# gfacciol/mgm

Measured on AMD Instinct MI355X. Metric: disparity-volumes/sec (W*H*L cost volume -> 8-dir MGM -> WTA+vfit), higher is better.
Workload: dtype f32

## Files before the change

mgm_amd/csrc/mgm_pass.hip:

```cpp
#include "mgm_pass_common.h"

namespace mgm {

template <int LPL, bool FH, bool WEIGHTED, int R>
__global__ void __launch_bounds__(R * 64) k_pass(const PassParams P)
{
    constexpr int LP = LPL * 64;
    constexpr int NS = (WEIGHTED && !FH) ? 2 : 1;
    using NbT = Nb<LPL, NS>;
    extern __shared__ __attribute__((aligned(16))) float smem[];
    float *ring = smem;
    float *ringm = smem + R * 2 * NS * LP;
    int *s_task = reinterpret_cast<int *>(ringm + R * 2);

    const int tid = threadIdx.x, lane = tid & 63;
    const int r = __builtin_amdgcn_readfirstlane(tid >> 6);
    if (tid == 0) *s_task = (int)atomicAdd(P.ticket, 1u);
    __syncthreads();
    const int2 tk = P.tasks[*s_task];
    const int vp = tk.x, band = tk.y;
    const int pass = vp & (kMaxDirs - 1);
    const PassVolume &V = P.vol[vp / kMaxDirs];
    const PassGeom &g = P.g[pass];
    const int NL = g.NL, LL = g.LL, L = P.L, MGM = P.MGM, form = g.form;
// ... 96 lines not shown
                        if (form == 0) combine_unit<LPL>(Cpf[u], nb_i, nb_s, nb_b, nb_f, MGM, FH, Lv);
                        else combine_unit<LPL>(Cpf[u], nb_f, nb_b, nb_s, nb_i, MGM, FH, Lv);
                    } else {
                        float D[4];
#pragma unroll
                        for (int k = 0; k < 4; k++) D[k] = V.w8[(long long)g.wplane[k] * P.npix + pix];
                        int rl = 0, rh = 0x7fffffff;
                        if (FH && V.rlo) {
                            rl = (int)V.rlo[pix] - P.dmin;
                            rh = (int)V.rhi[pix] - P.dmin;
                        }
                        if constexpr (!FH) {
                            if (form == 0) combine_whirsch<LPL>(Cpf[u], nb_i, nb_s, nb_b, nb_f, D, P1, P2, MGM, Lv);
                            else combine_whirsch<LPL>(Cpf[u], nb_f, nb_b, nb_s, nb_i, D, P1, P2, MGM, Lv);
                        } else {
                            if (form == 0) combine_wfh<LPL>(Cpf[u], nb_i, nb_s, nb_b, nb_f, D, P1, P2, MGM, lane, L, Lv, rl, rh);
                            else combine_wfh<LPL>(Cpf[u], nb_f, nb_b, nb_s, nb_i, D, P1, P2, MGM, lane, L, Lv, rl, rh);
                        }
                    }
                } else {
#pragma unroll
                    for (int k = 0; k < LPL; k++) Lv[k] = Cpf[u][k];
                }
                store_slab<LPL>(Lrb + pix * L, lane, L, exact, Lv);

                const float m = slab_min<LPL>(Lv);
                nb_i.m = m;
                if constexpr (!WEIGHTED) {
                    if constexpr (!FH) {
                        float N[LPL];
                        neighbour_min<LPL>(Lv, N);
                        const float cap = m + P2;
#pragma unroll
                        for (int k = 0; k < LPL; k++) nb_i.w[0][k] = fminf(fminf(Lv[k], N[k] + P1), cap);
                    } else {
#pragma unroll
                        for (int k = 0; k < LPL; k++) nb_i.w[0][k] = Lv[k];
                        fh_minconv<LPL>(nb_i.w[0], m, P1, P2, lane, L);
                    }
                } else {
#pragma unroll
                    for (int k = 0; k < LPL; k++) nb_i.w[0][k] = Lv[k];
                    if constexpr (!FH) neighbour_min<LPL>(Lv, nb_i.w[NS - 1]);
                }
                if (to_lds) {
                    float *dst = ring + (r * 2 + (i & 1)) * NS * LP + lane * LPL;
#pragma unroll
                    for (int q = 0; q < NS; q++)
#pragma unroll
                        for (int k = 0; k < LPL; k++) dst[q * LP + k] = nb_i.w[q][k];
                    if (lane == 0) ringm[r * 2 + (i & 1)] = m;
                }
                if (to_global) {
#pragma unroll
                    for (int q = 0; q < NS; q++)
                        store_slab_sc1<LPL>(hand_out + ((long long)i * NS + q) * LP, lane, nb_i.w[q]);
                    if (lane == 0)
                        __hip_atomic_store(reinterpret_cast<unsigned *>(handm_out + i), __builtin_bit_cast(unsigned, m),
                                           RLX_AGENT);
                    if (((i + 1) % CH) == 0 || i == LL - 1) {
                        asm volatile("s_waitcnt vmcnt(0)" ::: "memory");
                        if (lane == 0) __hip_atomic_store(prog_out, (unsigned)(i + 1), RLX_AGENT);
                    }
                }
            }

            issue_prefetch(s + PF, Cpf[u], Hpf[u]);

            lds_barrier();
        }
    }
}

__global__ void __launch_bounds__(256) k_selftest_div3(unsigned long long *nbad)
{
    unsigned long long bad = 0;
    const unsigned long long stride = (unsigned long long)gridDim.x * blockDim.x;
    for (unsigned long long b = (unsigned long long)blockIdx.x * blockDim.x + threadIdx.x; b < (1ull << 32); b += stride) {
        const float x = __builtin_bit_cast(float, (unsigned)b);
        const unsigned a = __builtin_bit_cast(unsigned, x / 3.0f);
        const unsigned q = __builtin_bit_cast(unsigned, div3_exact(x));
        const bool a_nan = (a & 0x7fffffffu) > 0x7f800000u, q_nan = (q & 0x7fffffffu) > 0x7f800000u;
        if (a != q && !(a_nan && q_nan)) bad++;
    }
    if (bad) atomicAdd(nbad, bad);
}
hipError_t launch_selftest_div3(unsigned long long *nbad, hipStream_t s)
{
    hipLaunchKernelGGL(k_selftest_div3, dim3(4096), dim3(256), 0, s, nbad);
    return hipGetLastError();
}

int pass_ns(bool fh, bool weighted) { return (weighted && !fh) ? 2 : 1; }
int pass_lpl(int L)
{
    const int lpl = (L + 63) / 64;
    if (lpl == 5) return 6;
    if (lpl == 7) return 8;
    if (lpl <= 8) return lpl;
    return lpl <= 12 ? 12 : (lpl <= 16 ? 16 : (lpl <= 24 ? 24 : 32));
}

hipError_t launch_pass(const PassParams &p, const PassKernelChoice &c, int ntasks, hipStream_t s)
{
    if (c.family != kPassFirst) return hipErrorInvalidValue;
    return lift<kR, 4>(c.R, [&](auto R) { return lift<32, 24, 16, 12, 8, 6, 4, 3, 2, 1>(c.LPL, [&](auto LPL) { return lift<1, 0>(c.WEIGHTED, [&](auto W) { return lift<0, 1>(c.FH, [&](auto FH) {
        if constexpr (pass_instance(LPL(), R())) {
            auto kern = k_pass<LPL(), FH() != 0, W() != 0, R()>;
            if (c.lds > 48 * 1024) {
                hipError_t e = hipFuncSetAttribute(reinterpret_cast<const void *>(kern), hipFuncAttributeMaxDynamicSharedMemorySize, c.lds);
                if (e != hipSuccess) return e;
            }
            hipLaunchKernelGGL(kern, dim3(ntasks), dim3(c.block), c.lds, s, p);
            return hipGetLastError();
        } else
            return hipErrorInvalidValue;
    }); }); }); });
}

}
```

mgm_amd/csrc/mgm_pass2.hip:

```cpp
#include <type_traits>

#include "mgm_pass_common.h"

namespace mgm {

typedef __attribute__((address_space(3))) void *lds_vptr;
typedef const __attribute__((address_space(1))) void *glb_vptr;

template <int AUX>
__device__ __forceinline__ void dma16(const float *src_lane, float *dst_base)
{
    __builtin_amdgcn_global_load_lds((glb_vptr)src_lane, (lds_vptr)dst_base, 16, 0, AUX);
}
template <int AUX>
__device__ __forceinline__ void dma4(const void *src_lane, void *dst_base)
{
    __builtin_amdgcn_global_load_lds((glb_vptr)src_lane, (lds_vptr)dst_base, 4, 0, AUX);
}
constexpr int AUX_SC1 = 16;

template <int N>
__device__ __forceinline__ void wait_vmcnt()
{
    static_assert(N >= 0 && N <= 63, "vmcnt is a 6-bit counter");
// ... 91 lines not shown
#endif
#ifndef MGM_P2_DEV
#define MGM_P2_DEV 0
#endif

#ifndef MGM_P2_TIMELINE
#define MGM_P2_TIMELINE 0
#endif
#ifndef MGM_P2_C8_NL
#define MGM_P2_C8_NL 1
#endif
#ifndef MGM_P2_C8_NC
#define MGM_P2_C8_NC (16 - MGM_P2_C8_NL)
#endif
#ifndef MGM_P2_MAXD
#define MGM_P2_MAXD 2
#endif
#ifndef MGM_P2_DEEPD
#define MGM_P2_DEEPD 4
#endif
#ifndef MGM_P2_PUBLAG
#define MGM_P2_PUBLAG 3
#endif
#ifndef MGM_P2_PUBEVERY
#define MGM_P2_PUBEVERY 4
#endif
#ifndef MGM_P2_LEAD
#define MGM_P2_LEAD 2
#endif
template <int LPL, int NS, bool HASM, int C8, int MAXD = MGM_P2_MAXD, int EXTRA = 0>
struct Plan {
    static constexpr int LP = LPL * 64;
    static constexpr int IPS = (LPL * 16 + 63) / 64;
    static constexpr int LPS = LPL * 4 * (C8 ? C8 : 1);
    static constexpr int LPD = C8 ? 64 / LPS : 1;
    static constexpr int NL = (LPL <= 4 && MGM_P2_NC > 7) ? (C8 ? MGM_P2_C8_NL : 2) : 1;
    static constexpr int NC = (LPL <= 4) ? (C8 ? MGM_P2_C8_NC : MGM_P2_NC) : 7;
    static constexpr int NCA = (NL == 2) ? NC / 2 : NC;
    static constexpr int NDMA = C8 ? (NC + LPD - 1) / LPD : NCA * IPS;
    static constexpr int nA = ((C8 && NL == 2) ? 0 : NDMA) + NS * IPS + (HASM ? 2 : 0) + EXTRA;
    static constexpr int nB = (C8 && NL == 2) ? NDMA : (NC - NCA) * IPS;
    static constexpr int cring_floats(int rdepth) { return C8 ? rdepth * NDMA * 256 : NC * rdepth * LP; }
    static constexpr int lds_floats3(int rt, int rdepth)
    {
        return NC * rt * NS * LP
               + NC * rt
               + rdepth * NS * LP
               + 2 * rdepth + 8 + 32
               + cring_floats(rdepth)
               + (C8 ? rdepth * 16 : 0)
               + EXTRA * rdepth * 64;
    }
    static constexpr bool fits(int rt, int rdepth, int d)
    {
        return d >= 2 && d <= rdepth - 1 && lds_floats3(rt, rdepth) * 4 <= ((C8 && LPL <= 4 && NS == 1) ? MGM_P2_LDS_KB : 160) * 1024 &&
               nA * (d - 1) <= 63 && nB * (d - 1) <= 63;
    }
    static constexpr int pick(int what)
    {
        const int rts[2] = {2, 2};
        const int rds[3] = {MAXD + 1, 4, 3};
        for (int a = 0; a < 2; a++)
            for (int b = 0; b < 3; b++)
                for (int d = MAXD; d >= 2; d--)
                    if (fits(rts[a], rds[b], d)) return what == 0 ? rts[a] : (what == 1 ? rds[b] : d);
        return 0;
    }
    static constexpr int RT = pick(0), RDEPTH = pick(1), D = pick(2);
    static constexpr int rd(int) { return RDEPTH; }
    static constexpr int lds_floats(int) { return lds_floats3(RT, RDEPTH); }
    static_assert(D >= 2, "no feasible pipeline depth");
    static_assert(!C8 || LPD >= 1, "a compact slab must fit a DMA piece");
    static_assert((RT & (RT - 1)) == 0, "RT must be a power of two");
};

template <int LPL, int MGM, bool FH>
__device__ __forceinline__ void combine_unit_E(const float (&C)[LPL], const float (&e1)[LPL], const float (&e2)[LPL],
                                               const float (&e3)[LPL], const float (&e4)[LPL], float (&out)[LPL])
{
    if constexpr (MGM == 2) {
#pragma unroll
        for (int k = 0; k < LPL; k++) out[k] = C[k] + (e1[k] + e2[k]);
    } else {
#pragma unroll
        for (int k = 0; k < LPL; k++) {
            float e = e1[k];
            if constexpr (MGM >= 3) e += e2[k];
            if constexpr (MGM >= 3) e += e3[k];
            if constexpr (MGM >= 4) e += e4[k];
            out[k] = C[k] + div_small<MGM>(e);
        }
    }
}

template <int LPL, int MGM>
__device__ __forceinline__ void combine_w2(const float (&C)[LPL], const Nb<LPL, 2> &n1, const Nb<LPL, 2> &n2, const Nb<LPL, 2> &n3,
                                           const Nb<LPL, 2> &n4, bool a1, bool a2, bool a3, bool a4, float (&out)[LPL])
{
#pragma unroll
    for (int k = 0; k < LPL; k++) {
        float e = a1 ? n1.w[1][k] : n1.w[0][k];
        if constexpr (MGM >= 2) e += a2 ? n2.w[1][k] : n2.w[0][k];
        if constexpr (MGM >= 3) e += a3 ? n3.w[1][k] : n3.w[0][k];
        if constexpr (MGM >= 4) e += a4 ? n4.w[1][k] : n4.w[0][k];
        out[k] = C[k] + div_small<MGM>(e);
    }
}

template <int LPL, bool FH, bool WEIGHTED, int MGM, int C8, bool DEEP, bool W2 = false>
struct P2Lds {
    static constexpr int NS = (W2 || (WEIGHTED && !FH)) ? 2 : 1;
    static constexpr bool pubE = W2 || (!WEIGHTED && !(FH && MGM == 2));
    using PL = Plan<LPL, NS, !pubE, C8, DEEP ? MGM_P2_DEEPD : MGM_P2_MAXD, W2 ? 1 : 0>;
    static constexpr int RD = PL::rd(PL::D);
    static constexpr int task_off = PL::NC * PL::RT * NS * PL::LP + RD * NS * PL::LP + PL::cring_floats(RD) + PL::NC * PL::RT + RD + RD;
};

template <int LPL, bool FH, bool WEIGHTED, int MGM, int C8, int SUBV, bool DEEP, bool XCDQ, bool W2 = false>
__device__ __forceinline__ void pass2_item(const PassParams &P, const int ticket)
{
    static_assert(!W2 || (!WEIGHTED && C8 && DEEP && SUBV == 1 && LPL <= 4), "two-valued weights: the compact kernels with deep rings");
    static_assert(!DEEP || (C8 && !WEIGHTED && (W2 || !(FH && MGM == 2))), "the deep rings exist for the compact kernels that publish E");
    static_assert(SUBV == 1 || (LPL == 4 && C8 == 1 && !WEIGHTED && !(FH && MGM == 2)), "volumes share a wave only in the compact unweighted kernels that publish E");
    static_assert(!W2 || C8 == 1, "two-valued weights: one byte per cost");
    constexpr int LANES = 64 / SUBV;
    constexpr int NS = (W2 || (WEIGHTED && !FH)) ? 2 : 1;
    constexpr bool pubE = W2 || (!WEIGHTED && !(FH && MGM == 2));
    constexpr bool TAGS = pubE;
    constexpr bool CFLAG = C8 && FH;
    constexpr bool CHMIN = LPL == 4 && SUBV == 1 && C8 == 1 && !WEIGHTED && !W2 && pubE;
    using PL = Plan<LPL, NS, !pubE, C8, DEEP ? MGM_P2_DEEPD : MGM_P2_MAXD, W2 ? 1 : 0>;
    static_assert(!W2 || PL::NL == 1, "two-valued weights: one loader wave");
    constexpr int LP = PL::LP, NC = PL::NC, NCA = PL::NCA, D = PL::D, IPS = PL::IPS;
    constexpr int LPS = PL::LPS, LPD = PL::LPD, NDMA = PL::NDMA;
    constexpr int LPW = NCA;
    constexpr int RD = PL::rd(D);
    constexpr int RT = PL::RT;
    using NbT = Nb<LPL, NS>;

    extern __shared__ __attribute__((aligned(16))) float smem[];
    float *Tring = smem;
    float *Hring = Tring + NC * RT * NS * LP;
    float *Cring = Hring + RD * NS * LP;
    float *Tm = Cring + PL::cring_floats(RD);
    float *Hm = Tm + NC * RT;
    unsigned *Hprog = reinterpret_cast<unsigned *>(Hm + RD);
    int *s_task = reinterpret_cast<int *>(smem + P2Lds<LPL, FH, WEIGHTED, MGM, C8, DEEP, W2>::task_off);
    unsigned *Cflag = reinterpret_cast<unsigned *>(s_task + 40);
    unsigned *Wring = Cflag + RD * 16;

    const int tid = threadIdx.x, lane = tid & 63;
    const int wave = __builtin_amdgcn_readfirstlane(tid >> 6);
    const int2 tk = P.tasks[ticket];
    const int vp = tk.x, band = tk.y & 0xffff, strip = (tk.y >> 16) & 0xff;
    const bool plain_out = XCDQ && ((tk.y >> 24) & 1) != 0;
    const int pass = vp & (kMaxDirs - 1);
    const int vgrp = (vp / kMaxDirs) * SUBV;
    const PassVolume &V = P.vol[vgrp];
#if MGM_P2_DEV
    unsigned long long *dbg = P.dbg ? P.dbg + (long long)ticket * 16 : nullptr;
    const int xflags = P.xflags;
#else
    constexpr unsigned long long *dbg = nullptr;
    constexpr int xflags = 0;
#endif
    if (dbg && tid == 0) dbg[0] = wall_clock64();
    const PassGeom &g = P.g[pass];
    const int NLn = g.NL, LL = g.LL, L = P.L, form = g.form;
    const float P1 = P.P1, P2 = P.P2;
    const int SL = g.slope;
    const bool strips = TAGS && g.nstrips == 2;
    const bool mirror = strips && strip == 1;
    const long long istep = mirror ? -g.istep : g.istep;
    const long long gbase = mirror ? g.base + (long long)(LL - 1) * g.istep : g.base;
    const int W = !strips ? LL : min(LL, (strip == 0 ? g.split : LL - g.split) + NC - 1);
    const int nsteps = ((W + 1 + SL * (NC - 1)) + 2) / 3 * 3;
    const bool from_global = band > 0;

    constexpr int NSLP = NS * LP;
    const long long hslab = (long long)(vp / kMaxDirs) * P.hand_vstride + g.hand_base;
    float *hand_out = TAGS ? P.hand + (hslab + (long long)band * LL) * NSLP : P.hand + ((long long)(vp * 2 + (band & 1)) * P.LLmax) * NSLP;
    float *handm_out = P.handm + (long long)(vp * 2 + (band & 1)) * P.LLmax;
    const float *hand_in = TAGS ? P.hand + (hslab + (long long)(band > 0 ? band - 1 : 0) * LL) * NSLP
                                : P.hand + ((long long)(vp * 2 + ((band + 1) & 1)) * P.LLmax) * NSLP;
    const float *handm_in = P.handm + (long long)(vp * 2 + ((band + 1) & 1)) * P.LLmax;
    unsigned *prog_out = P.prog + vp * P.maxbands + band;
    const unsigned *prog_in = from_global ? prog_out - 1 : prog_out;

    const unsigned tag_in = P.hand_tag[pass], tag_out = tag_in;

    if (wave >= NC) {
        const int wl = wave - NC;
        const int r0 = wl == 0 ? 0 : NCA;
        unsigned known = 0;
        bool dead = false;
        unsigned long long n_slow = 0, t_slow = 0, n_spin = 0, t_ret = 0, t_bar = 0, t_iss = 0, tl_wait = 0;
        (void)tl_wait;
        (void)n_slow;
        (void)n_spin;

        constexpr int NPIECE = C8 ? NDMA : LPW;
        const float *cptr[NPIECE];
        int ci[NPIECE];
        const long long cstride = C8 ? (istep * L * C8) / 4 : istep * L;
#pragma unroll
        for (int q = 0; q < NPIECE; q++) {
            int r = C8 ? q * LPD + lane / LPS : r0 + q;
            r = r < NC ? r : NC - 1;
            int j = band * NC + r;
            j = j < NLn ? j : NLn - 1;
            if constexpr (C8 && SUBV > 1) {
                constexpr int CPV = LPS / SUBV;
                const int chunk = lane % LPS;
// ... 345 lines not shown
                    }
                } else {
                    const float *src = c_src0 + cslot * LP;
#pragma unroll
                    for (int k = 0; k < LPL; k++) Cv[k] = src[k];
                }
                const bool interior = has_prev && i >= 1 && i <= LL - 2;
                if (prof) {
                    asm volatile("s_waitcnt lgkmcnt(0)" ::: "memory");
                    asm volatile("" : "+v"(Cv[0]), "+v"(X.w[0][0]));
                    ph[0] += clock64() - c0;
                }
                const unsigned long long c1 = prof ? clock64() : 0;
                const NbT &nb_same = SLOPE == 2 ? Z : X;
                const NbT &nb_back = SLOPE == 2 ? Y : Z;
                const NbT &nb_fwd = X;
                if (interior) {
                    if constexpr (W2) {
                        const unsigned wm = (unsigned)__builtin_amdgcn_readfirstlane((int)Wring[cslot * 64 + r]);
                        const bool a0 = (wm >> wb[0]) & 1u, a1 = (wm >> wb[1]) & 1u, a2 = (wm >> wb[2]) & 1u, a3 = (wm >> wb[3]) & 1u;
                        if constexpr (FORM == 0) combine_w2<LPL, MGM>(Cv, nb_i, nb_same, nb_back, nb_fwd, a0, a1, a2, a3, Lv);
                        else combine_w2<LPL, MGM>(Cv, nb_fwd, nb_back, nb_same, nb_i, a0, a1, a2, a3, Lv);
                    } else if constexpr (!WEIGHTED) {
                        if constexpr (pubE) {
                            if constexpr (FORM == 0)
                                combine_unit_E<LPL, MGM, FH>(Cv, nb_i.w[0], nb_same.w[0], nb_back.w[0], nb_fwd.w[0], Lv);
                            else
                                combine_unit_E<LPL, MGM, FH>(Cv, nb_fwd.w[0], nb_back.w[0], nb_same.w[0], nb_i.w[0], Lv);
                        } else {
                            if constexpr (FORM == 0) combine_unit<LPL>(Cv, nb_i, nb_same, nb_back, nb_fwd, MGM, FH, Lv);
                            else combine_unit<LPL>(Cv, nb_fwd, nb_back, nb_same, nb_i, MGM, FH, Lv);
                        }
                    } else {
                        float Dw[4];
#pragma unroll
                        for (int k = 0; k < 4; k++) Dw[k] = V.w8[(long long)g.wplane[k] * P.npix + pix];
                        int rl = 0, rh = 0x7fffffff;
                        if (FH && V.rlo) {
                            rl = (int)V.rlo[pix] - P.dmin;
                            rh = (int)V.rhi[pix] - P.dmin;
                        }
                        if constexpr (!FH) {
                            if constexpr (FORM == 0)
                                combine_whirsch<LPL>(Cv, nb_i, nb_same, nb_back, nb_fwd, Dw, P1, P2, MGM, Lv);
                            else
                                combine_whirsch<LPL>(Cv, nb_fwd, nb_back, nb_same, nb_i, Dw, P1, P2, MGM, Lv);
                        } else {
                            if (MGM == 2 && P.fh2_ragged) {
                                if constexpr (FORM == 0) combine_fh2_ragged<LPL>(Cv, nb_i, nb_same, P1, P2, lane, P.Lreal, rl, rh, Lv);
                                else combine_fh2_ragged<LPL>(Cv, nb_fwd, nb_back, P1, P2, lane, P.Lreal, rl, rh, Lv);
                            } else if constexpr (FORM == 0)
                                combine_wfh<LPL>(Cv, nb_i, nb_same, nb_back, nb_fwd, Dw, P1, P2, MGM, lane, P.Lreal, Lv, rl, rh);
                            else
                                combine_wfh<LPL>(Cv, nb_fwd, nb_back, nb_same, nb_i, Dw, P1, P2, MGM, lane, P.Lreal, Lv, rl, rh);
                        }
                    }
                } else {
#pragma unroll
                    for (int k = 0; k < LPL; k++) Lv[k] = Cv[k];
                }
                if (prof) {
                    asm volatile("" : "+v"(Lv[0]), "+v"(Lv[LPL - 1]));
                    ph[1] += clock64() - c1;
                }
                const unsigned long long c2 = prof ? clock64() : 0;
                if (!(xflags & 1)) {
#ifdef MGM_P2_XFLAG16
                    float *q = Lrb + ((xflags & 16) ? (pix & 255) : pix) * L + (lane % LANES) * LPL;
#else
                    float *q = q_here;
#endif
#pragma unroll
                    for (int k = 0; k < LPL; k++) q[k] = Lv[k];
                }
                float m;
                if constexpr (CHMIN) {
                    m = Lv[0];
#pragma unroll
                    for (int k = 1; k < LPL; k++) m = fminf(m, Lv[k]);
                    m = dpp_min_row_shr1(m, m);
                    m = dpp_min_row_shr2(m, m);
                    m = dpp_min_row_shr4(m, m);
                    if (P.min_k != 0 && (lane & 7) == 7)
                        *reinterpret_cast<float *>((long long)(reinterpret_cast<unsigned long long>(q_here) >> 5) + P.min_k) = m;
                    m = dpp_min_row_shr8(m, m);
                    m = dpp_min_bcast15(m, m);
                    m = dpp_min_bcast31(m, m);
                    m = readlane_f(m, 63);
                } else if constexpr (SUBV == 1) {
                    m = slab_min<LPL>(Lv);
                } else {
                    m = Lv[0];
#pragma unroll
                    for (int k = 1; k < LPL; k++) m = fminf(m, Lv[k]);
                    m = dpp_min_row_shr1(m, m);
                    m = dpp_min_row_shr2(m, m);
                    m = dpp_min_row_shr4(m, m);
                    m = dpp_min_row_shr8(m, m);
                    if constexpr (SUBV == 2) m = dpp_min_bcast15(m, m);
                    m = __shfl(m, lane | (LANES - 1));
                }
                nb_i.m = m;
                if (prof) {
                    float mm = m;
                    asm volatile("" : "+v"(mm));
                    ph[2] += clock64() - c2;
                }
                const unsigned long long c3 = prof ? clock64() : 0;
                if constexpr (W2) {
                    const float P1a = V.p1a, P2a = V.p2a;
                    if constexpr (!FH) {
                        float N[LPL];
                        neighbour_min<LPL>(Lv, N);
                        const float cap = m + P2, capa = m + P2a;
#pragma unroll
                        for (int k = 0; k < LPL; k++) {
                            nb_i.w[0][k] = fminf(fminf(Lv[k], N[k] + P1), cap) - m;
                            nb_i.w[1][k] = fminf(fminf(Lv[k], N[k] + P1a), capa) - m;
                        }
                    } else {
#pragma unroll
                        for (int k = 0; k < LPL; k++) nb_i.w[0][k] = nb_i.w[1][k] = Lv[k];
                        unsigned sw = 0;
                        const unsigned need = ((unsigned)__builtin_amdgcn_readfirstlane((int)Wring[cslot * 64 + r]) >> (8 + 2 * pass)) & 3u;
                        if (need & 1u) fh_minconv<LPL, false, 1>(nb_i.w[0], m, P1, P2, lane, P.Lreal, sw);
                        if (need & 2u) fh_minconv<LPL, false, 1>(nb_i.w[1], m, P1a, P2a, lane, P.Lreal, sw);
#pragma unroll
                        for (int k = 0; k < LPL; k++) {
                            nb_i.w[0][k] -= m;
                            nb_i.w[1][k] -= m;
                        }
                    }
                } else if constexpr (!WEIGHTED) {
                    if constexpr (!FH) {
                        float N[LPL];
                        neighbour_min<LPL>(Lv, N, SUBV > 1 && lane % LANES == 0, SUBV > 1 && lane % LANES == LANES - 1);
                        const float cap = m + P2;
#pragma unroll
                        for (int k = 0; k < LPL; k++) nb_i.w[0][k] = fminf(fminf(Lv[k], N[k] + P1), cap);
                    } else {
#pragma unroll
                        for (int k = 0; k < LPL; k++) nb_i.w[0][k] = Lv[k];
                        unsigned sw = 0;
                        fh_minconv<LPL, false, SUBV>(nb_i.w[0], m, P1, P2, lane, P.Lreal, sw);
                        if (prof) { fh_sweeps += sw; fh_max = sw > fh_max ? sw : fh_max; fh_n++; fh_rep += sw > 2; }
                    }
                    if constexpr (pubE) {
#pragma unroll
                        for (int k = 0; k < LPL; k++) nb_i.w[0][k] = MGM == 2 ? (nb_i.w[0][k] - m) * 0.5f : nb_i.w[0][k] - m;
                    }
                } else {
#pragma unroll
                    for (int k = 0; k < LPL; k++) nb_i.w[0][k] = Lv[k];
                    if constexpr (!FH) neighbour_min<LPL>(Lv, nb_i.w[NS - 1]);
                }
                if (prof) {
                    asm volatile("" : "+v"(nb_i.w[0][0]), "+v"(nb_i.w[0][LPL - 1]));
                    ph[3] += clock64() - c3;
                }
                const unsigned long long c4 = prof ? clock64() : 0;
                if (to_lds) {
                    float *dst = t_dst0 + (i & (RT - 1)) * NSLP;
#pragma unroll
                    for (int q = 0; q < NS; q++)
#pragma unroll
                        for (int k = 0; k < LPL; k++) dst[q * LP + k] = nb_i.w[q][k];
                    if constexpr (!pubE)
                        if (lane == 0) Tm[r * RT + (i & (RT - 1))] = m;
                }
                if (prof) {
                    asm volatile("s_waitcnt lgkmcnt(0)" ::: "memory");
                    ph[4] += clock64() - c4;
                }
                if constexpr (TAGS) {
                    if (to_global) {
#pragma unroll
                        for (int q = 0; q < NS; q++) {
                            float tagged[LPL];
#pragma unroll
                            for (int k = 0; k < LPL; k++)
                                tagged[k] = __builtin_bit_cast(float, (__builtin_bit_cast(unsigned, nb_i.w[q][k]) & 0x7fffffffu) | tag_out);
                            float *hs = hand_out + ((long long)(mirror ? LL - 1 - i : i) * NS + q) * LP;
                            if constexpr (XCDQ) {
                                if (plain_out) store_slab_plain<LPL>(hs, lane, tagged);
                                else store_slab_sc1_wide<LPL>(hs, lane, tagged);
                            } else
                                store_slab_sc1_wide<LPL>(hs, lane, tagged);
                        }
                    }
                } else if (to_global) {
#pragma unroll
                    for (int q = 0; q < NS; q++)
                        store_slab_sc1_wide<LPL>(hand_out + ((long long)i * NS + q) * LP, lane, nb_i.w[q]);
                    if constexpr (!pubE)
                        if (lane == 0) st_sc1_x1(handm_out + i, m);
                    constexpr int SPS = 1 + NS * sc1_store_count<LPL>();
                    constexpr int PUBLAG = (63 / SPS) < MGM_P2_PUBLAG ? (63 / SPS) : MGM_P2_PUBLAG;
                    constexpr int PUBEVERY = MGM_P2_PUBEVERY;
                    if (i == LL - 1) {
                        wait_vmcnt<0>();
                        if (lane == 0) __hip_atomic_store(prog_out, (unsigned)LL, RLX_AGENT);
                    } else if (((i - PUBLAG + 1) % PUBEVERY) == 0 && i - PUBLAG >= 0) {
                        wait_vmcnt<PUBLAG * SPS>();
                        if (lane == 0) __hip_atomic_store(prog_out, (unsigned)(i - PUBLAG + 1), RLX_AGENT);
                    }
                }
            }
        };

        int cslot = 0;
        unsigned long long t_cbar = 0;
        step_barrier((xflags & 8) != 0);
        for (int s = 0; s < nsteps; s += 3) {
            step(s, cslot, wA, wB, wC);
            cslot = cslot + 1 == RD ? 0 : cslot + 1;
            const unsigned long long t0 = (dbg && r == NC / 2) ? wall_clock64() : 0;
            step_barrier((xflags & 8) != 0);
            if (dbg && r == NC / 2) t_cbar += wall_clock64() - t0;
            step(s + 1, cslot, wB, wC, wA);
            cslot = cslot + 1 == RD ? 0 : cslot + 1;
            step_barrier((xflags & 8) != 0);
            step(s + 2, cslot, wC, wA, wB);
            cslot = cslot + 1 == RD ? 0 : cslot + 1;
            step_barrier((xflags & 8) != 0);
        }
        if (dbg && r == NC / 2 && lane == 0) {
            dbg[14] = t_cbar * 3;
// ... 79 lines not shown
```

mgm_amd/csrc/mgm_pass_common.h:

```cpp
#pragma once
#include <type_traits>

#include "mgm_device.h"
#include "mgm_planner.h"

namespace mgm {

template <int... Vs, class F>
static hipError_t lift(int v, F f)
{
    hipError_t e = hipErrorInvalidValue;
    (void)((v == Vs && ((e = f(std::integral_constant<int, Vs>{})), true)) || ...);
    return e;
}

constexpr int PF = 4;
constexpr int CH = 8;
constexpr unsigned SPIN_LIMIT = 1u << 22;

#define RLX_AGENT __ATOMIC_RELAXED, __HIP_MEMORY_SCOPE_AGENT

__device__ __forceinline__ void lds_barrier()
{
    asm volatile("s_waitcnt lgkmcnt(0)" ::: "memory");
// ... 115 lines not shown
            const double tp = row == 0 ? t1 : (row == 1 ? t2 : t3);
            s = dmin(s, row <= 2 ? tp + (double)(16 - li) * Rd : inf);
        } else if constexpr (GROUPS == 2) {
            const double t1 = readlane_f64(s, 16), t3 = readlane_f64(s, 48);
            s = dmin(s, (row & 1) ? inf : (row == 0 ? t1 : t3) + (double)(16 - li) * Rd);
        }
    }
    s -= P1d;
    if (P1 > 0.0f) {
        double B = (double)__builtin_bit_cast(float, (__builtin_bit_cast(unsigned, P1) & 0x7f800000u) + 0x00800000u);
        for (int it = 0; it < 64; it++) {
            const bool reach = s < inf && s >= B;
            if (__builtin_amdgcn_ballot_w64(reach) == 0ull) break;
            const double magic = B * 805306368.0;
            const double r = (s + magic) - magic;
            s = reach ? r : s;
            B += B;
        }
    }
    return fminf(a, (float)s);
}

template <int LPL, bool FWD, int GROUPS = 1>
__device__ __forceinline__ float fh_careful(float a, float P1, int lane_in)
{
    constexpr int GL = 64 / GROUPS;
    int lane = lane_in;
    asm volatile("" : "+v"(lane));
    asm volatile("" : "+v"(P1));
    const float R = (float)LPL * P1, inf = f_inf();
    const int li = lane & 15, row = lane >> 4, lg = lane % GL;
    float b = a;
#pragma unroll
    for (int q = 0; q < LPL; q++) b = b + P1;
    float s = FWD ? dpp_shr1(b, inf) : dpp_shl1(b, inf);
    s = (FWD ? lg == 0 : lg == GL - 1) ? inf : s;
    auto cut2 = [&](float off, float &p1, float &p2) {
        p1 = fminf(off, 4.0f * R);
        p2 = off - p1;
    };
    if constexpr (FWD) {
        s = dpp_min_row_shr1(s, s + R);
        s = dpp_min_row_shr2(s, s + 2.0f * R);
        s = dpp_min_row_shr4(s, s + 4.0f * R);
        s = dpp_min_row_shr8(s, (s + 4.0f * R) + 4.0f * R);
        if constexpr (GROUPS <= 2) {
            float p1, p2;
            cut2((float)(li + 1) * R, p1, p2);
            const bool on = GROUPS == 1 ? row >= 1 : (row & 1);
            float t = dpp_add_bcast15(s, on ? p1 : inf);
            t = t + (on ? p2 : 0.0f);
            s = fminf(s, t);
        }
        if constexpr (GROUPS == 1) {
            const float off = (float)(li + 1 + (row == 3 ? 16 : 0)) * R;
            const float p1 = fminf(off, 4.0f * R), p2 = fminf(off - p1, 12.0f * R), p3 = (off - p1) - p2;
            const bool on = row >= 2;
            float t = dpp_add_bcast31(s, on ? p1 : inf);
            t = (t + (on ? p2 : 0.0f)) + (on ? p3 : 0.0f);
            s = fminf(s, t);
        }
    } else {
        s = dpp_min_row_shl1(s, s + R);
        s = dpp_min_row_shl2(s, s + 2.0f * R);
        s = dpp_min_row_shl4(s, s + 4.0f * R);
        s = dpp_min_row_shl8(s, (s + 4.0f * R) + 4.0f * R);
        auto add16 = [&](float x) { return (x + 4.0f * R) + 12.0f * R; };
        float p1, p2;
        cut2((float)(16 - li) * R, p1, p2);
        if constexpr (GROUPS == 1) {
            const float t3 = readlane_f(s, 48);
            const float t2 = fminf(readlane_f(s, 32), add16(t3));
            const float t1 = fminf(readlane_f(s, 16), add16(t2));
            const float tp = row == 0 ? t1 : (row == 1 ? t2 : t3);
            s = fminf(s, row <= 2 ? (tp + p1) + p2 : inf);
        } else if constexpr (GROUPS == 2) {
            const float t1 = readlane_f(s, 16), t3 = readlane_f(s, 48);
            s = fminf(s, (row & 1) ? inf : ((row == 0 ? t1 : t3) + p1) + p2);
        }
    }
    return fminf(a, s);
}

template <int LPL, bool FWD, int GROUPS = 1>
__device__ __forceinline__ void fh_scan(float (&M)[LPL], float P1, int lane, unsigned &sweeps)
{
    static_assert(GROUPS == 1 || GROUPS == 2 || GROUPS == 4, "lane groups of 64, 32 or 16");
    constexpr int GL = 64 / GROUPS;
    constexpr int K0 = FWD ? 0 : LPL - 1;
    constexpr int K1 = FWD ? LPL - 1 : 0;
    constexpr int DK = FWD ? 1 : -1;
    const float rampP = (float)LPL * P1;

    auto origin = [&](bool again) {
        float a = M[K0];
        if (again) asm volatile("" : "+v"(a));
#pragma unroll
        for (int q = 1; q < LPL; q++) a = fminf(M[K0 + q * DK], a + P1);
        return a;
    };
    const float a = origin(false);

    const int li = lane & 15, row = lane >> 4;
    const float r1 = rampP, r2 = 2.0f * rampP, r4 = 4.0f * rampP, r8 = 8.0f * rampP, r16 = 16.0f * rampP;
    float c = a;
    if constexpr (FWD) {
        c = dpp_min_row_shr1(c, c + r1);
        c = dpp_min_row_shr2(c, c + r2);
        c = dpp_min_row_shr4(c, c + r4);
        c = dpp_min_row_shr8(c, c + r8);
        if constexpr (GROUPS <= 2) {
            const float offA = (GROUPS == 1 ? row >= 1 : (row & 1)) ? (float)(li + 1) * rampP : f_inf();
            c = fminf(c, dpp_add_bcast15(c, offA));
        }
        if constexpr (GROUPS == 1) {
            const float offB = row >= 2 ? (float)(li + 1 + (row == 3 ? 16 : 0)) * rampP : f_inf();
            c = fminf(c, dpp_add_bcast31(c, offB));
        }
    } else {
        c = dpp_min_row_shl1(c, c + r1);
        c = dpp_min_row_shl2(c, c + r2);
        c = dpp_min_row_shl4(c, c + r4);
        c = dpp_min_row_shl8(c, c + r8);
        if constexpr (GROUPS == 1) {
            const float offA0 = row == 0 ? (float)(16 - li) * rampP : f_inf();
            const float offA2 = row == 2 ? (float)(16 - li) * rampP : f_inf();
            const float offB = row <= 1 ? (float)(32 - lane) * rampP : f_inf();
            c = fminf(fminf(c, readlane_f(c, 16) + offA0), readlane_f(c, 48) + offA2);
            c = fminf(c, readlane_f(c, 32) + offB);
        } else if constexpr (GROUPS == 2) {
            const float t1 = readlane_f(c, 16), t3 = readlane_f(c, 48);
            const float tp = row == 0 ? t1 : t3;
            const float offD = (row & 1) ? f_inf() : (float)(16 - li) * rampP;
            c = fminf(c, tp + offD);
        }
        (void)r16;
    }
    const float p1edge = (FWD ? lane % GL == 0 : lane % GL == GL - 1) ? f_inf() : P1;
    float f[LPL];
    int boosted = 0;
    for (int it = 0; it < 70; it++) {
        const float cin = FWD ? dpp_add_wave_shr1(c, p1edge) : dpp_add_wave_shl1(c, p1edge);
        f[K0] = fminf(M[K0], cin);
#pragma unroll
        for (int q = 1; q < LPL; q++) f[K0 + q * DK] = fminf(M[K0 + q * DK], f[K0 + (q - 1) * DK] + P1);
        const bool same = (f[K1] == c);
        c = f[K1];
        sweeps++;
        if (__builtin_amdgcn_ballot_w64(!same) == 0ull) break;
        if (boosted == 0) {
            boosted = 1;
#ifdef MGM_FH_NOREPAIR
            break;
#endif
            c = fh_careful<LPL, FWD, GROUPS>(origin(true), P1, lane);
        } else if (boosted == 1) {
            boosted = 2;
            c = fh_repair<LPL, FWD, GROUPS>(origin(true), P1, lane);
        }
    }
#pragma unroll
    for (int k = 0; k < LPL; k++) M[k] = f[k];
}

template <int LPL, bool FULL = false, int GROUPS = 1>
__device__ __forceinline__ void fh_minconv(float (&M)[LPL], float m, float P1, float P2, int lane, int L, unsigned &sweeps)
{
    constexpr int GL = 64 / GROUPS;
    fh_scan<LPL, true, GROUPS>(M, P1, lane, sweeps);
    if (L < GL * LPL) {
#pragma unroll
        for (int k = 0; k < LPL; k++) M[k] = ((lane % GL) * LPL + k < L) ? M[k] : f_inf();
    }
    fh_scan<LPL, false, GROUPS>(M, P1, lane, sweeps);
    if (P2 < f_inf()) {
        const float cap = m + P2;
#pragma unroll
        for (int k = 0; k < LPL; k++) M[k] = fminf(M[k], cap);
    }
}
template <int LPL, bool FWD, int GROUPS, int NK>
__device__ __forceinline__ void fh_scan_multi(float (&M)[NK][LPL], const float (&P1)[NK], int lane, unsigned &sweeps)
{
    static_assert(GROUPS == 4, "rows of 16 lanes: the only user is the range-proportional pass kernel");
    constexpr int GL = 64 / GROUPS;
    constexpr int K0 = FWD ? 0 : LPL - 1;
    constexpr int K1 = FWD ? LPL - 1 : 0;
    constexpr int DK = FWD ? 1 : -1;
    float c[NK], t[NK], rp[NK];
#pragma unroll
    for (int k = 0; k < NK; k++) c[k] = M[k][K0];
#pragma unroll
    for (int q = 1; q < LPL; q++)
#pragma unroll
        for (int k = 0; k < NK; k++) c[k] = fminf(M[k][K0 + q * DK], c[k] + P1[k]);
#pragma unroll
    for (int k = 0; k < NK; k++) rp[k] = (float)LPL * P1[k];
#pragma unroll
    for (int st = 0; st < 4; st++) {
#pragma unroll
        for (int k = 0; k < NK; k++) t[k] = c[k] + (float)(1 << st) * rp[k];
        if constexpr (FWD) {
            if (st == 0) dpp_min_row_shr1_n<NK>(c, t);
            else if (st == 1) dpp_min_row_shr2_n<NK>(c, t);
            else if (st == 2) dpp_min_row_shr4_n<NK>(c, t);
            else dpp_min_row_shr8_n<NK>(c, t);
        } else {
            if (st == 0) dpp_min_row_shl1_n<NK>(c, t);
            else if (st == 1) dpp_min_row_shl2_n<NK>(c, t);
            else if (st == 2) dpp_min_row_shl4_n<NK>(c, t);
            else dpp_min_row_shl8_n<NK>(c, t);
        }
    }
    const bool edge = FWD ? lane % GL == 0 : lane % GL == GL - 1;
    float pe[NK], cin[NK], f[NK][LPL];
#pragma unroll
    for (int k = 0; k < NK; k++) pe[k] = edge ? f_inf() : P1[k];
    if constexpr (FWD) dpp_add_wave_shr1_n<NK>(cin, c, pe);
    else dpp_add_wave_shl1_n<NK>(cin, c, pe);
#pragma unroll
    for (int k = 0; k < NK; k++) f[k][K0] = fminf(M[k][K0], cin[k]);
#pragma unroll
    for (int q = 1; q < LPL; q++)
#pragma unroll
        for (int k = 0; k < NK; k++) f[k][K0 + q * DK] = fminf(M[k][K0 + q * DK], f[k][K0 + (q - 1) * DK] + P1[k]);
    bool same = true;
#pragma unroll
    for (int k = 0; k < NK; k++) same = same && (f[k][K1] == c[k]);
    sweeps += NK;
    if (__builtin_amdgcn_ballot_w64(!same) == 0ull) {
#pragma unroll
        for (int k = 0; k < NK; k++)
#pragma unroll
            for (int q = 0; q < LPL; q++) M[k][q] = f[k][q];
    } else {
#pragma unroll
        for (int k = 0; k < NK; k++) fh_scan<LPL, FWD, GROUPS>(M[k], P1[k], lane, sweeps);
    }
}
template <int LPL, int GROUPS, int NK>
__device__ __forceinline__ void fh_minconv_multi(float (&M)[NK][LPL], const float (&m)[NK], const float (&P1)[NK], const float (&P2)[NK], int lane,
                                                 unsigned &sweeps)
{
    fh_scan_multi<LPL, true, GROUPS, NK>(M, P1, lane, sweeps);
    fh_scan_multi<LPL, false, GROUPS, NK>(M, P1, lane, sweeps);
#pragma unroll
    for (int k = 0; k < NK; k++) {
        const float cap = m[k] + P2[k];
#pragma unroll
        for (int q = 0; q < LPL; q++) M[k][q] = fminf(M[k][q], cap);
    }
}
template <int LPL, bool FULL = false>
__device__ __forceinline__ void fh_minconv(float (&M)[LPL], float m, float P1, float P2, int lane, int L)
{
    unsigned sweeps = 0;
    fh_minconv<LPL, FULL>(M, m, P1, P2, lane, L, sweeps);
}

__device__ __forceinline__ float div3_exact(float x)
{
    const float c = 0x1.555556p-2f;
    const float q0 = x * c;
    const float r = __builtin_fmaf(-3.0f, q0, x);
    const float q = __builtin_fmaf(r, c, q0);
    return __builtin_amdgcn_div_fixupf(q, 3.0f, x);
}
template <int N>
__device__ __forceinline__ float div_small(float e)
{
    static_assert(N >= 1 && N <= 4, "MGM is 1..4");
    if constexpr (N == 1) return e;
    else if constexpr (N == 2) return e * 0.5f;
    else if constexpr (N == 3) return div3_exact(e);
    else return e * 0.25f;
}
__device__ __forceinline__ float div_small_rt(float e, int n)
{
    return n == 1 ? e : (n == 2 ? e * 0.5f : (n == 3 ? div3_exact(e) : e * 0.25f));
}

template <int LPL, int NS>
struct Nb {
    float w[NS][LPL];
    float m;
};

template <int LPL>
__device__ __forceinline__ void combine_unit(const float (&C)[LPL], const Nb<LPL, 1> &n1, const Nb<LPL, 1> &n2,
                                             const Nb<LPL, 1> &n3, const Nb<LPL, 1> &n4, int MGM, bool FH,
                                             float (&out)[LPL])
{
    if (MGM == 2) {
        if (!FH) {
#pragma unroll
            for (int k = 0; k < LPL; k++) {
                float e = 0.0f;
                e += (n1.w[0][k] - n1.m) * 0.5f;
                e += (n2.w[0][k] - n2.m) * 0.5f;
                out[k] = C[k] + e;
            }
        } else {
#pragma unroll
            for (int k = 0; k < LPL; k++) out[k] = C[k] + (((n1.w[0][k] - n1.m) + n2.w[0][k]) - n2.m) * 0.5f;
        }
        return;
    }
#pragma unroll
    for (int k = 0; k < LPL; k++) {
        float e;
        if (!FH) {
            e = 0.0f;
            e += n1.w[0][k] - n1.m;
        } else {
            e = n1.w[0][k] - n1.m;
        }
        if (MGM >= 2) e += n2.w[0][k] - n2.m;
        if (MGM >= 3) e += n3.w[0][k] - n3.m;
        if (MGM >= 4) e += n4.w[0][k] - n4.m;
        out[k] = C[k] + div_small_rt(e, MGM);
    }
}

template <int LPL>
__device__ __forceinline__ float hirsch_w_term(const Nb<LPL, 2> &n, int k, float p1, float p2)
{
    const float t = fminf(fminf(n.w[0][k], n.w[1][k] + p1), n.m + p2);
    return t - n.m;
}
template <int LPL>
__device__ __forceinline__ void combine_whirsch(const float (&C)[LPL], const Nb<LPL, 2> &n1, const Nb<LPL, 2> &n2,
                                                const Nb<LPL, 2> &n3, const Nb<LPL, 2> &n4, const float (&D)[4],
                                                float P1, float P2, int MGM, float (&out)[LPL])
{
    const float a1 = P1 * D[0], b1 = P2 * D[0], a2 = P1 * D[1], b2 = P2 * D[1];
    const float a3 = P1 * D[2], b3 = P2 * D[2], a4 = P1 * D[3], b4 = P2 * D[3];
#pragma unroll
    for (int k = 0; k < LPL; k++) {
        float e = 0.0f;
        e += hirsch_w_term<LPL>(n1, k, a1, b1);
        if (MGM >= 2) e += hirsch_w_term<LPL>(n2, k, a2, b2);
        if (MGM >= 3) e += hirsch_w_term<LPL>(n3, k, a3, b3);
        if (MGM >= 4) e += hirsch_w_term<LPL>(n4, k, a4, b4);
        out[k] = C[k] + div_small_rt(e, MGM);
    }
}
template <int LPL, bool FULL = false>
__device__ __forceinline__ void combine_wfh(const float (&C)[LPL], const Nb<LPL, 1> &n1, const Nb<LPL, 1> &n2,
                                            const Nb<LPL, 1> &n3, const Nb<LPL, 1> &n4, const float (&D)[4], float P1,
                                            float P2, int MGM, int lane, int L, float (&out)[LPL], int rl = 0,
// ... 74 lines not shown
```

Baseline: 176.3.

## Fuse forward/backward min-convolution scans and pack exact div-by-3 into float2 ops

Introduces a fused FH min-convolution that computes the in-lane prefix once and propagates only cross-lane carries, avoiding recomputation of the per-lane min chain on every sweep iteration. It is enabled for compact full-horizontal kernels without XCD queueing. Separately, the exact divide-by-3 used in MGM=3 combines is vectorized into packed two-wide FMA/mul operations, with the self-test extended to check the packed variant. The min-store pointer is also cast to the global address space so the compiler can emit a global store instead of a flat one. The fused scan reorganizes the carry and repair logic, which risks numerical or convergence differences if the carry handling is subtly wrong.

```diff
diff --git a/mgm_amd/csrc/mgm_pass.hip b/mgm_amd/csrc/mgm_pass.hip
--- a/mgm_amd/csrc/mgm_pass.hip
+++ b/mgm_amd/csrc/mgm_pass.hip
@@ -202,6 +202,14 @@
         const unsigned q = __builtin_bit_cast(unsigned, div3_exact(x));
         const bool a_nan = (a & 0x7fffffffu) > 0x7f800000u, q_nan = (q & 0x7fffffffu) > 0x7f800000u;
         if (a != q && !(a_nan && q_nan)) bad++;
+        const float y = __builtin_bit_cast(float, (unsigned)b ^ 0xAAAAAAAAu);
+        const mgm_f2 q2 = div3_exact2(mgm_f2{x, y});
+        const unsigned ay = __builtin_bit_cast(unsigned, y / 3.0f);
+        const float q2x = q2.x, q2y = q2.y;
+        const unsigned qx = __builtin_bit_cast(unsigned, q2x), qy = __builtin_bit_cast(unsigned, q2y);
+        const bool ay_nan = (ay & 0x7fffffffu) > 0x7f800000u;
+        if (a != qx && !(a_nan && (qx & 0x7fffffffu) > 0x7f800000u)) bad++;
+        if (ay != qy && !(ay_nan && (qy & 0x7fffffffu) > 0x7f800000u)) bad++;
     }
     if (bad) atomicAdd(nbad, bad);
 }
diff --git a/mgm_amd/csrc/mgm_pass2.hip b/mgm_amd/csrc/mgm_pass2.hip
--- a/mgm_amd/csrc/mgm_pass2.hip
+++ b/mgm_amd/csrc/mgm_pass2.hip
@@ -197,13 +197,23 @@
 #pragma unroll
         for (int k = 0; k < LPL; k++) out[k] = C[k] + (e1[k] + e2[k]);
     } else {
-#pragma unroll
-        for (int k = 0; k < LPL; k++) {
+        auto sum = [&](int k) {
             float e = e1[k];
             if constexpr (MGM >= 3) e += e2[k];
             if constexpr (MGM >= 3) e += e3[k];
             if constexpr (MGM >= 4) e += e4[k];
-            out[k] = C[k] + div_small<MGM>(e);
+            return e;
+        };
+        if constexpr (MGM == 3 && LPL % 2 == 0) {
+#pragma unroll
+            for (int k = 0; k + 1 < LPL; k += 2) {
+                const mgm_f2 q = div3_exact2(mgm_f2{sum(k), sum(k + 1)});
+                out[k] = C[k] + q.x;
+                out[k + 1] = C[k + 1] + q.y;
+            }
+        } else {
+#pragma unroll
+            for (int k = 0; k < LPL; k++) out[k] = C[k] + div_small<MGM>(sum(k));
         }
     }
 }
@@ -212,13 +222,23 @@
 __device__ __forceinline__ void combine_w2(const float (&C)[LPL], const Nb<LPL, 2> &n1, const Nb<LPL, 2> &n2, const Nb<LPL, 2> &n3,
                                            const Nb<LPL, 2> &n4, bool a1, bool a2, bool a3, bool a4, float (&out)[LPL])
 {
-#pragma unroll
-    for (int k = 0; k < LPL; k++) {
+    auto sum = [&](int k) {
         float e = a1 ? n1.w[1][k] : n1.w[0][k];
         if constexpr (MGM >= 2) e += a2 ? n2.w[1][k] : n2.w[0][k];
         if constexpr (MGM >= 3) e += a3 ? n3.w[1][k] : n3.w[0][k];
         if constexpr (MGM >= 4) e += a4 ? n4.w[1][k] : n4.w[0][k];
-        out[k] = C[k] + div_small<MGM>(e);
+        return e;
+    };
+    if constexpr (MGM == 3 && LPL % 2 == 0) {
+#pragma unroll
+        for (int k = 0; k + 1 < LPL; k += 2) {
+            const mgm_f2 q = div3_exact2(mgm_f2{sum(k), sum(k + 1)});
+            out[k] = C[k] + q.x;
+            out[k + 1] = C[k + 1] + q.y;
+        }
+    } else {
+#pragma unroll
+        for (int k = 0; k < LPL; k++) out[k] = C[k] + div_small<MGM>(sum(k));
     }
 }
 
@@ -244,6 +264,7 @@
     constexpr bool TAGS = pubE;
     constexpr bool CFLAG = C8 && FH;
     constexpr bool CHMIN = LPL == 4 && SUBV == 1 && C8 == 1 && !WEIGHTED && !W2 && pubE;
+    constexpr bool FUSED = FH && C8 != 0 && !XCDQ;
     using PL = Plan<LPL, NS, !pubE, C8, DEEP ? MGM_P2_DEEPD : MGM_P2_MAXD, W2 ? 1 : 0>;
     static_assert(!W2 || PL::NL == 1, "two-valued weights: one loader wave");
     constexpr int LP = PL::LP, NC = PL::NC, NCA = PL::NCA, D = PL::D, IPS = PL::IPS;
@@ -755,7 +776,7 @@
                     m = dpp_min_row_shr2(m, m);
                     m = dpp_min_row_shr4(m, m);
                     if (P.min_k != 0 && (lane & 7) == 7)
-                        *reinterpret_cast<float *>((long long)(reinterpret_cast<unsigned long long>(q_here) >> 5) + P.min_k) = m;
+                        *(__attribute__((address_space(1))) float *)((long long)(reinterpret_cast<unsigned long long>(q_here) >> 5) + P.min_k) = m;
                     m = dpp_min_row_shr8(m, m);
                     m = dpp_min_bcast15(m, m);
                     m = dpp_min_bcast31(m, m);
@@ -815,7 +836,8 @@
 #pragma unroll
                         for (int k = 0; k < LPL; k++) nb_i.w[0][k] = Lv[k];
                         unsigned sw = 0;
-                        fh_minconv<LPL, false, SUBV>(nb_i.w[0], m, P1, P2, lane, P.Lreal, sw);
+                        if constexpr (FUSED) fh_minconv_fused<LPL, SUBV>(nb_i.w[0], m, P1, P2, lane, P.Lreal, sw);
+                        else fh_minconv<LPL, false, SUBV>(nb_i.w[0], m, P1, P2, lane, P.Lreal, sw);
                         if (prof) { fh_sweeps += sw; fh_max = sw > fh_max ? sw : fh_max; fh_n++; fh_rep += sw > 2; }
                     }
                     if constexpr (pubE) {
diff --git a/mgm_amd/csrc/mgm_pass_common.h b/mgm_amd/csrc/mgm_pass_common.h
--- a/mgm_amd/csrc/mgm_pass_common.h
+++ b/mgm_amd/csrc/mgm_pass_common.h
@@ -221,25 +221,9 @@
     return fminf(a, s);
 }
 
-template <int LPL, bool FWD, int GROUPS = 1>
-__device__ __forceinline__ void fh_scan(float (&M)[LPL], float P1, int lane, unsigned &sweeps)
-{
-    static_assert(GROUPS == 1 || GROUPS == 2 || GROUPS == 4, "lane groups of 64, 32 or 16");
-    constexpr int GL = 64 / GROUPS;
-    constexpr int K0 = FWD ? 0 : LPL - 1;
-    constexpr int K1 = FWD ? LPL - 1 : 0;
-    constexpr int DK = FWD ? 1 : -1;
-    const float rampP = (float)LPL * P1;
-
-    auto origin = [&](bool again) {
-        float a = M[K0];
-        if (again) asm volatile("" : "+v"(a));
-#pragma unroll
-        for (int q = 1; q < LPL; q++) a = fminf(M[K0 + q * DK], a + P1);
-        return a;
-    };
-    const float a = origin(false);
-
+template <int LPL, bool FWD, int GROUPS>
+__device__ __forceinline__ float fh_guess(float a, float rampP, int lane)
+{
     const int li = lane & 15, row = lane >> 4;
     const float r1 = rampP, r2 = 2.0f * rampP, r4 = 4.0f * rampP, r8 = 8.0f * rampP, r16 = 16.0f * rampP;
     float c = a;
@@ -275,6 +259,28 @@
         }
         (void)r16;
     }
+    return c;
+}
+
+template <int LPL, bool FWD, int GROUPS = 1>
+__device__ __forceinline__ void fh_scan(float (&M)[LPL], float P1, int lane, unsigned &sweeps)
+{
+    static_assert(GROUPS == 1 || GROUPS == 2 || GROUPS == 4, "lane groups of 64, 32 or 16");
+    constexpr int GL = 64 / GROUPS;
+    constexpr int K0 = FWD ? 0 : LPL - 1;
+    constexpr int K1 = FWD ? LPL - 1 : 0;
+    constexpr int DK = FWD ? 1 : -1;
+    const float rampP = (float)LPL * P1;
+
+    auto origin = [&](bool again) {
+        float a = M[K0];
+        if (again) asm volatile("" : "+v"(a));
+#pragma unroll
+        for (int q = 1; q < LPL; q++) a = fminf(M[K0 + q * DK], a + P1);
+        return a;
+    };
+    const float a = origin(false);
+    float c = fh_guess<LPL, FWD, GROUPS>(a, rampP, lane);
     const float p1edge = (FWD ? lane % GL == 0 : lane % GL == GL - 1) ? f_inf() : P1;
     float f[LPL];
     int boosted = 0;
@@ -318,6 +324,71 @@
         for (int k = 0; k < LPL; k++) M[k] = fminf(M[k], cap);
     }
 }
+__device__ __forceinline__ float fmin3f(float a, float b, float c) { return fminf(fminf(a, b), c); }
+
+template <int LPL, bool FWD, int GROUPS>
+__device__ __forceinline__ float fh_fused_carries(const float (&g)[LPL], float (&r)[LPL], float P1, int lane, unsigned &sweeps)
+{
+    constexpr int GL = 64 / GROUPS;
+    constexpr int K0 = FWD ? 0 : LPL - 1;
+    constexpr int K1 = FWD ? LPL - 1 : 0;
+    constexpr int DK = FWD ? 1 : -1;
+    auto origin = [&]() {
+        float a = g[K1];
+        asm volatile("" : "+v"(a));
+        return a;
+    };
+    float c = fh_guess<LPL, FWD, GROUPS>(g[K1], (float)LPL * P1, lane);
+    const float p1edge = (FWD ? lane % GL == 0 : lane % GL == GL - 1) ? f_inf() : P1;
+    int boosted = 0;
+    for (int it = 0; it < 70; it++) {
+        r[K0] = FWD ? dpp_add_wave_shr1(c, p1edge) : dpp_add_wave_shl1(c, p1edge);
+#pragma unroll
+        for (int q = 1; q < LPL; q++) r[K0 + q * DK] = r[K0 + (q - 1) * DK] + P1;
+        const float fl = fminf(g[K1], r[K1]);
+        const bool same = (fl == c);
+        c = fl;
+        sweeps++;
+        if (__builtin_amdgcn_ballot_w64(!same) == 0ull) break;
+        if (boosted == 0) {
+            boosted = 1;
+#ifdef MGM_FH_NOREPAIR
+            break;
+#endif
+            c = fh_careful<LPL, FWD, GROUPS>(origin(), P1, lane);
+        } else if (boosted == 1) {
+            boosted = 2;
+            c = fh_repair<LPL, FWD, GROUPS>(origin(), P1, lane);
+        }
+    }
+    return c;
+}
+template <int LPL, int GROUPS = 1>
+__device__ __forceinline__ void fh_minconv_fused(float (&M)[LPL], float m, float P1, float P2, int lane, int L, unsigned &sweeps)
+{
+    constexpr int GL = 64 / GROUPS;
+    float g[LPL], r[LPL];
+    g[0] = M[0];
+#pragma unroll
+    for (int k = 1; k < LPL; k++) g[k] = fminf(M[k], g[k - 1] + P1);
+    float fl = fh_fused_carries<LPL, true, GROUPS>(g, r, P1, lane, sweeps);
+    if (L < GL * LPL) {
+#pragma unroll
+        for (int k = 0; k < LPL; k++) {
+            g[k] = ((lane % GL) * LPL + k < L) ? fminf(g[k], r[k]) : f_inf();
+            r[k] = f_inf();
+        }
+        fl = g[LPL - 1];
+    }
+    g[LPL - 1] = fl;
+#pragma unroll
+    for (int k = LPL - 2; k >= 0; k--) g[k] = fmin3f(g[k], r[k], g[k + 1] + P1);
+    fh_fused_carries<LPL, false, GROUPS>(g, r, P1, lane, sweeps);
+    const float cap = m + P2;
+#pragma unroll
+    for (int k = 0; k < LPL; k++) M[k] = fmin3f(g[k], r[k], cap);
+}
+
 template <int LPL, bool FWD, int GROUPS, int NK>
 __device__ __forceinline__ void fh_scan_multi(float (&M)[NK][LPL], const float (&P1)[NK], int lane, unsigned &sweeps)
 {
@@ -405,6 +476,17 @@
     const float q = __builtin_fmaf(r, c, q0);
     return __builtin_amdgcn_div_fixupf(q, 3.0f, x);
 }
+typedef float mgm_f2 __attribute__((ext_vector_type(2)));
+__device__ __forceinline__ mgm_f2 div3_exact2(mgm_f2 x)
+{
+    float kc, km3, k3;
+    asm volatile("s_mov_b32 %0, 0x3eaaaaab\n\ts_mov_b32 %1, 0xc0400000\n\ts_mov_b32 %2, 0x40400000" : "=s"(kc), "=s"(km3), "=s"(k3));
+    const mgm_f2 c = {kc, kc}, m3 = {km3, km3};
+    const mgm_f2 q0 = x * c;
+    const mgm_f2 r = __builtin_elementwise_fma(m3, q0, x);
+    const mgm_f2 q = __builtin_elementwise_fma(r, c, q0);
+    return mgm_f2{__builtin_amdgcn_div_fixupf(q.x, k3, x.x), __builtin_amdgcn_div_fixupf(q.y, k3, x.y)};
+}
 template <int N>
 __device__ __forceinline__ float div_small(float e)
 {
```

New measurement: 171.2. 2.9% lower.
